# c-zhou/oatk

Measured on AMD Instinct MI355X. Metric: HiFi Gbases/s through syncasm (syncmer+syncerr) at k=1001 s=31, higher is better.
Workload: dtype u64

## Files before the change

oatk_amd/csrc/api_ec.inc:

```
#include "../../include/oatk_hip_ec.h"
#include "ec.hpp"
#include "ec_wave.hpp"
#include "ec_heavy.hpp"
#include "ec_fused.hpp"
#include "ecgraph.hpp"
#include "ec_seq.hpp"
#include <rocprim/device/device_run_length_encode.hpp>
#include <rocprim/device/device_select.hpp>

struct EcState {
    DevBuf idx_p, idx_n, arc_v, arc_w, arc_ls, arc_cov, arc_del, conv;
    DevBuf scm_del, err_del, vtx_hs_off, vtx_mpos;
    DevBuf copy_n, seg, keep_all, n_blocks, n_blocks64, blk_off, work, out, path_pool, cursor, todo, todo2, slabs, big_slabs, os_slabs;
    DevBuf hyb_slabs[16];
    hipStream_t aux[5] = {nullptr, nullptr, nullptr, nullptr, nullptr};
    hipEvent_t aux_ev[5] = {nullptr, nullptr, nullptr, nullptr, nullptr}, fork_ev = nullptr;
    DevBuf new_n, new_n64, new_off, new_k, new_m, new_s, stats;
    DevBuf live32, live64, live_off, larc, lidx_p, lidx_n;
    DevBuf cov, fwd, key_id, key_sorted, val_occ, occ, occ_off, cov64;
    uint64_t n_vtx = 0, new_tot = 0;
    uint64_t stats_h[12] = {0};
    uint64_t n_work = 0;
    bool done = false;
    DevBuf g_keys, g_keys2, g_ukeys, g_counts, g_nruns, g_nout, g_nout64, g_outoff, g_akey, g_aval, g_skey, g_sval, g_comp, g_flags, g_huge;
    DevBuf g_dist, g_dist2, g_cnt64, g_runoff, g_runls;
    DevBuf g_big, g_keep, g_other, g_lkeys, g_ldist, g_val2, g_wgt2, g_runcov, g_head, g_hpos, g_iota, g_segk, g_segv;
    uint32_t light_c = 0;
    uint64_t g_n_vtx = 0, g_n_arc = 0;
    bool graph_resident = false;
    bool global = false, marked = false;
    uint64_t n_global = 0, imp_used = 0;
    DevBuf g_l2g, g_kid, g_gcov, g_gs;
    bool keep_seq = false;
    bool seq_kept = false, cseq_done = false;
    bool seq_global = false;
    DevBuf slot_w, slot_w64, slot_off, slots, qend, sblk, clen, cbytes, cbytes64, coff, cseq;
    uint64_t cseq_bytes = 0;
};

static uint64_t ec_n_vtx(oatk_hip_ctx *ctx) { return ctx->ec && ctx->ec->global? ctx->ec->n_global : ctx->n_scm_total; }
static const uint64_t *ec_chains(oatk_hip_ctx *ctx) { return ctx->ec && ctx->ec->global? ctx->ec->g_kid.as<uint64_t>() : ctx->pos_kid.as<uint64_t>(); }

static void ec_state_free(oatk_hip_ctx *ctx)
{
    if (!ctx->ec) return;
    EcState *e = ctx->ec;
    for (int i = 0; i < 5; ++i) { if (e->aux[i]) (void) hipStreamDestroy(e->aux[i]); if (e->aux_ev[i]) (void) hipEventDestroy(e->aux_ev[i]); }
    if (e->fork_ev) (void) hipEventDestroy(e->fork_ev);
    delete e;
    ctx->ec = nullptr;
}

static int ec_buffer(oatk_hip_ctx *ctx, int which, const void **d_ptr, uint64_t *bytes)
{
    EcState *e = ctx->ec;
    if (e && which >= OATK_BUF_EG_IDX_P && which <= OATK_BUF_EG_ARC_COMP) {
        if (!e->graph_resident) { ctx->err = "EC graph requested before oatk_hip_ec_graph"; return OATK_E_STATE; }
        const uint64_t gv = e->g_n_vtx, ga = e->g_n_arc;
        switch (which) {
            case OATK_BUF_EG_IDX_P: *d_ptr = e->idx_p.p, *bytes = 2 * gv * 8; break;
            case OATK_BUF_EG_IDX_N: *d_ptr = e->idx_n.p, *bytes = 2 * gv * 4; break;
            case OATK_BUF_EG_ARC_V: *d_ptr = e->arc_v.p, *bytes = ga * 8; break;
            case OATK_BUF_EG_ARC_W: *d_ptr = e->arc_w.p, *bytes = ga * 8; break;
            case OATK_BUF_EG_ARC_LS: *d_ptr = e->arc_ls.p, *bytes = ga * 4; break;
            case OATK_BUF_EG_ARC_COV: *d_ptr = e->arc_cov.p, *bytes = ga * 4; break;
            default: *d_ptr = e->g_comp.p, *bytes = ga; break;
        }
        return OATK_OK;
    }
    if (e && (which == OATK_BUF_EC_VTX_SRC || (which == OATK_BUF_EC_ERR_DEL && !e->done))) {
        if (!e->marked) { ctx->err = "vertex sources / marks requested before oatk_hip_ec_mark"; return OATK_E_STATE; }
        if (which == OATK_BUF_EC_VTX_SRC) *d_ptr = e->vtx_hs_off.p, *bytes = e->n_vtx * 8;
        else *d_ptr = e->err_del.p, *bytes = e->n_vtx;
        return OATK_OK;
    }
// ... 576 lines not shown
{
    using namespace oatk;
    if (!ctx) return OATK_E_NODEV;
    if (!ctx->ec || !ctx->ec->marked) { ctx->err = "oatk_hip_ec_export_kmers needs oatk_hip_ec_mark"; return OATK_E_STATE; }
    if (stride % 16 || stride < (uint32_t) ((ctx->K + 3) / 4 + 8)) { ctx->err = "k-mer stride must be a multiple of 16 and hold the k-mer + 8 bytes"; return OATK_E_ARG; }
    CK(hipSetDevice(ctx->device));
    EcState *e = ctx->ec;
    if (n) hipLaunchKernelGGL(ecw_export_kmer_kernel, dim3((unsigned) n), dim3(64), 0, ctx->stream, n, d_ids, e->vtx_hs_off.as<uint64_t>(), e->vtx_mpos.as<uint32_t>(),
                              ctx->hoco_s.as<uint8_t>(), ctx->K, stride, d_out, d_rev);
    CK(hipStreamSynchronize(ctx->stream));
    CK(hipGetLastError());
    return OATK_OK;
}

extern "C" int oatk_hip_ec_import_kmers(oatk_hip_ctx *ctx, const uint32_t *d_ids, const uint8_t *d_rev, const uint8_t *d_kmers, uint64_t n, uint32_t stride)
{
    using namespace oatk;
    if (!ctx) return OATK_E_NODEV;
    if (!ctx->ec || !ctx->ec->marked) { ctx->err = "oatk_hip_ec_import_kmers needs oatk_hip_ec_mark"; return OATK_E_STATE; }
    if (stride % 16 || stride < (uint32_t) ((ctx->K + 3) / 4 + 8)) { ctx->err = "k-mer stride must be a multiple of 16 and hold the k-mer + 8 bytes"; return OATK_E_ARG; }
    CK(hipSetDevice(ctx->device));
    EcState *e = ctx->ec;
    if (n && !ctx->hoco_s.p) { ctx->err = "oatk_hip_ec_import_kmers: this batch has no hoco strings to put k-mers behind"; return OATK_E_STATE; }
    const uint64_t base = ((ctx->seq_bytes / 4 + 128) + 15) & ~15ULL;
    if (e->imp_used + n * stride > ctx->import_reserve) { ctx->err = "imported k-mers exceed the reserve behind the hoco strings (oatk_hip_ec_reserve_import before the scan)"; return OATK_E_NOMEM; }
    if (n) {
        CK(hipMemcpyAsync(ctx->hoco_s.as<uint8_t>() + base + e->imp_used, d_kmers, n * stride, hipMemcpyDeviceToDevice, ctx->stream));
        hipLaunchKernelGGL(ecw_import_kmer_kernel, dim3((unsigned) ((n + 255) / 256)), dim3(256), 0, ctx->stream, n, d_ids, d_rev, base + e->imp_used, stride,
                           e->vtx_hs_off.as<uint64_t>(), e->vtx_mpos.as<uint32_t>());
        e->imp_used += n * stride;
    }
    CK(hipStreamSynchronize(ctx->stream));
    CK(hipGetLastError());
    return OATK_OK;
}

extern "C" int oatk_hip_ec_reserve_import(oatk_hip_ctx *ctx, uint64_t bytes)
{
    if (!ctx) return OATK_E_NODEV;
    ctx->import_reserve = bytes < (1u << 20)? (1u << 20) : (bytes + 15) & ~15ULL;
    return OATK_OK;
}

struct EcKnobs {
    int heavy = -1;
    bool stages = false;
    bool serial_tiers = false;
    int32_t step_budget = 1000;
    int32_t min_nw = 0;
    int32_t heavy_cap2 = 0;
    int32_t heavy_fl = 0;
    int32_t waves = 32;
    bool assemble_walk = false;
};
static EcKnobs ec_knobs_read()
{
    EcKnobs k;
    auto num = [](const char *n, int32_t lo, int32_t dflt) { const char *e = getenv(n); return e && atoi(e) >= lo? (int32_t) atoi(e) : dflt; };
    { const char *e = getenv("OATK_DEBUG_EC_HEAVY"); k.heavy = e && (e[0] == '0' || e[0] == '1') && !e[1]? e[0] - '0' : -1; }
    k.stages = getenv("OATK_DEBUG_EC_STAGES") != nullptr;
    { const char *e = getenv("OATK_DEBUG_EC_SERIAL_TIERS"); k.serial_tiers = e && e[0] == '1'; }
    k.step_budget = num("OATK_DEBUG_EC_STEP_BUDGET", 1, 1000);
    k.min_nw = num("OATK_DEBUG_EC_FUSED_MIN_NW", 2, 0);
    k.heavy_cap2 = num("OATK_DEBUG_EC_HEAVY_CAP2", 1, 0), k.heavy_fl = num("OATK_DEBUG_EC_HEAVY_FL", 64, 0) & ~7;
    k.waves = num("OATK_DEBUG_EC_WAVES", 1, 32);
    { const char *e = getenv("OATK_DEBUG_EC_ASSEMBLE_WALK"); k.assemble_walk = e && e[0] == '1'; }
    return k;
}

namespace oatk {

static const int32_t EC_CAP_T0 = 3072;
static const int32_t EC_CAP_T1 = 16384;
static const int32_t EC_ARC_BUDGET = 512;

struct EcTier { int32_t cap_t, cap_c, cap_w, cap_path, cap_f; uint64_t bytes, slab; bool usable, hybrid; int wpb; };

static int32_t ec_cap_c(int32_t cap_t, int K) { return cap_t + cap_t / 8 + 2 * K + 64; }

static int32_t ec_band_cap(int32_t bwmax, double max_edist)
{
    int64_t ct = max_edist > 0? (int64_t) floor((double) bwmax / max_edist) : 0x3FFFFFFF;
    while (ct > 0 && (int32_t) ceil((double) ct * max_edist) > bwmax) --ct;
    return (int32_t) (ct > 60000? 60000 : ct);
}

static uint64_t ec_wg_per_cu(uint64_t bytes)
{
    const uint64_t n = 160 * 1024 / (bytes + 256);
    return n > 16? 16 : (n? n : 1);
}

static EcTier ec_lds_tier(int32_t cap_t, int32_t cap_path, int32_t cap_f, bool hybrid, double max_edist, int K)
{
    EcTier t;
    const int32_t bw = (int32_t) (cap_t * max_edist) + 1;
    t.cap_t = cap_t, t.cap_w = 2 * (bw > EC_MIN_ERR_BASE? bw : EC_MIN_ERR_BASE) + 12, t.cap_c = ec_cap_c(cap_t, K);
    t.hybrid = hybrid;
    if (hybrid) {
        t.cap_path = t.cap_c, t.cap_f = 1 << 20;
        t.bytes = (uint64_t) ecw_lds_words_hybrid(t.cap_t, t.cap_c, t.cap_w) * 4;
        t.slab = ecw_slab_bytes_hybrid(t.cap_path, t.cap_f);
    } else {
        t.cap_path = cap_path, t.cap_f = cap_f;
        t.bytes = (uint64_t) ecw_scratch_words(t.cap_t, t.cap_c, t.cap_w, t.cap_path, t.cap_f, false) * 4;
        t.slab = 0;
    }
    t.usable = t.bytes <= 64 * 1024;
    t.wpb = ECW_WPB * t.bytes <= 64 * 1024? ECW_WPB : 1;
    return t;
}

static uint64_t ec_tier_waves(const EcTier &t, int32_t per_cu_max, int n_cu)
{
    uint64_t per_cu = ec_wg_per_cu((uint64_t) t.wpb * t.bytes) * (uint64_t) t.wpb;
    if (per_cu > (uint64_t) per_cu_max) per_cu = (uint64_t) per_cu_max / (uint64_t) t.wpb * (uint64_t) t.wpb;
    return (uint64_t) n_cu * (per_cu? per_cu : (uint64_t) t.wpb);
}

// ... 345 lines not shown
    int used_aux = 0;
    if (side_by_side) {
        { int rc = ec_route(ctx, e, n_work, rt, routed, sizeof(routed)); if (rc) return rc; }
        { int rc = ec_fork_side_streams(ctx, e); if (rc) return rc; }
        for (int tier = LAST - 1; tier >= 1; --tier) {
            if (!T[tier].usable || !routed[tier]) continue;
            hipStream_t st = e->aux[used_aux];
            CK(hipStreamWaitEvent(st, e->fork_ev, 0));
            { int rc = launch(tier, list[tier], routed[tier], st, true, tier == 1? 2 * (uint64_t) ctx->n_cu : 0); if (rc) return rc; }
            CK(hipEventRecord(e->aux_ev[used_aux], st));
            ++used_aux;
            done[tier] = routed[tier];
        }
    }
    const int first_tier = side_by_side || T[0].usable? 0 : next_usable(0);
    { int rc = launch(first_tier, nullptr, 0, ctx->stream, side_by_side); if (rc) return rc; }
    bool waited_aux = used_aux == 0;
    for (int round = 0; ; ++round) {
        CK(hipMemcpyAsync(cnts, cur, sizeof(cnts), hipMemcpyDeviceToHost, ctx->stream));
        CK(hipStreamSynchronize(ctx->stream));
        if (round == 0) n_big = cnts[1] + cnts[2] + routed[3];
        bool any = false;
        for (int tier = first_tier + 1; tier <= LAST; ++tier) {
            if (!T[tier].usable || cnts[tier] <= done[tier]) continue;
            { int rc = launch(tier, list[tier] + done[tier], cnts[tier] - done[tier], ctx->stream, false); if (rc) return rc; }
            done[tier] = cnts[tier];
            any = true;
        }
        if (!any && waited_aux) break;
        if (!waited_aux) { for (int i = 0; i < used_aux; ++i) CK(hipStreamWaitEvent(ctx->stream, e->aux_ev[i], 0)); waited_aux = true; }
    }
    return OATK_OK;
}

}

extern "C" int oatk_hip_ec_correct(oatk_hip_ctx *ctx, double max_edist)
{
    using namespace oatk;
    if (!ctx) return OATK_E_NODEV;
    if (!ctx->ec || !ctx->ec->marked) { ctx->err = "oatk_hip_ec_correct needs oatk_hip_ec_mark"; return OATK_E_STATE; }
    CK(hipSetDevice(ctx->device));
    EcState *e = ctx->ec;
    e->done = false, e->cseq_done = false;
    const bool keep_seq = e->keep_seq;
    e->seq_kept = false;
    const EcKnobs kn = ec_knobs_read();
    EC_VIEWS();
    EcLive lv;
    bool graph_branches = true;
    {
        uint64_t n_live = 0;
        EENSURE(g_flags, 64);
        CK(hipMemsetAsync(e->g_flags.as<uint32_t>() + 8, 0, 8, ctx->stream));
        EENSURE(live32, (na + 1) * 4); EENSURE(lidx_p, (2 * nv + 1) * 4); EENSURE(lidx_n, (2 * nv + 1) * 4);
        if (na) hipLaunchKernelGGL(ec_live_flag_kernel, blocks(na), dim3(256), 0, ctx->stream, na, (const uint8_t *) e->arc_del.p, e->live32.as<uint32_t>());
        { int rc = ec_exclusive_scan_u32(ctx, e, e->live32, e->live64, e->live_off, na, &n_live); if (rc) return rc; }
        if (n_live >= 0xFFFFFFFFULL) { ctx->err = "error correction: more than 2^32 live arcs"; return OATK_E_ARG; }
        EENSURE(larc, (n_live + 1) * sizeof(EcLiveArc));
        hipLaunchKernelGGL(ec_live_idx_kernel, blocks(2 * nv), dim3(256), 0, ctx->stream, 2 * nv, e->idx_p.as<uint64_t>(), e->idx_n.as<uint32_t>(),
                           e->live_off.as<uint64_t>(), e->lidx_p.as<uint32_t>(), e->lidx_n.as<uint32_t>(), e->g_flags.as<uint32_t>() + 9);
        if (na) hipLaunchKernelGGL(ec_live_arc_kernel, blocks(na), dim3(256), 0, ctx->stream, na, (const uint8_t *) e->arc_del.p, e->live_off.as<uint64_t>(),
                                   e->arc_w.as<uint64_t>(), e->arc_ls.as<uint32_t>(), e->vtx_hs_off.as<uint64_t>(), e->vtx_mpos.as<uint32_t>(),
                                   e->lidx_p.as<uint32_t>(), e->lidx_n.as<uint32_t>(), e->larc.as<EcLiveArc>(), e->g_flags.as<uint32_t>() + 8);
        uint32_t fl[2] = {0, 0};
        CK(hipMemcpyAsync(fl, e->g_flags.as<uint32_t>() + 8, 8, hipMemcpyDeviceToHost, ctx->stream));
        CK(hipStreamSynchronize(ctx->stream));
        const uint32_t no_src = fl[0];
        graph_branches = fl[1] != 0;
        if (no_src && ctx->n_occ) { ctx->err = "error correction: a live vertex has no k-mer on this shard (import it: oatk_hip_ec_import_kmers)"; return OATK_E_STATE; }
        lv.idx_p = e->lidx_p.as<uint32_t>(), lv.idx_n = e->lidx_n.as<uint32_t>(), lv.arc = e->larc.as<EcLiveArc>();
    }

    EENSURE(n_blocks, (nr + 1) * 4);
    const dim3 rblocks((unsigned) ((nr + ECR_READS_PER_BLOCK - 1) / ECR_READS_PER_BLOCK > 0? (nr + ECR_READS_PER_BLOCK - 1) / ECR_READS_PER_BLOCK : 1));
    hipLaunchKernelGGL(ec_count_blocks_wave_kernel, rblocks, dim3(256), 0, ctx->stream, rd, (const uint8_t *) e->scm_del.p, e->n_blocks.as<uint32_t>());
    uint64_t n_work = 0;
    { int rc = ec_exclusive_scan_u32(ctx, e, e->n_blocks, e->n_blocks64, e->blk_off, nr, &n_work); if (rc) return rc; }
    EENSURE(work, (n_work + 1) * sizeof(EcWork)); EENSURE(out, (n_work + 1) * sizeof(EcBlockOut));
    e->n_work = n_work;
    EENSURE(new_n, (nr + 1) * 4); EENSURE(copy_n, (nr + 1) * 4); EENSURE(seg, (n_work + 1) * sizeof(EcSeg)); EENSURE(keep_all, nr + 1);
    hipLaunchKernelGGL(ec_list_blocks_wave_kernel, rblocks, dim3(256), 0, ctx->stream, rd, lv, (const uint8_t *) e->scm_del.p, e->blk_off.as<uint64_t>(), e->work.as<EcWork>(), e->copy_n.as<uint32_t>(),
                       e->seg.as<EcSeg>(), e->keep_all.as<uint8_t>());
    if (keep_seq) {
        uint64_t slot_words = 0;
        EENSURE(slot_w, (n_work + 1) * 4); EENSURE(qend, (n_work + 1) * 4);
        if (n_work) hipLaunchKernelGGL(ec_slot_words_kernel, blocks(n_work), dim3(256), 0, ctx->stream, e->work.as<EcWork>(), n_work, max_edist, e->slot_w.as<uint32_t>());
        { int rc = ec_exclusive_scan_u32(ctx, e, e->slot_w, e->slot_w64, e->slot_off, n_work, &slot_words); if (rc) return rc; }
        EENSURE(slots, (slot_words + 4) * 4);
    }
    t_end(ctx, OATK_T_EC_MARK);
    t_begin(ctx, OATK_T_EC_SOLVE);

    const bool heavy = kn.heavy < 0? graph_branches : kn.heavy != 0;
    uint64_t pool_cap = 2 * nocc + (uint64_t) 16384 * ECW_POOL_CHUNK + 4096;
    EENSURE(cursor, 512); EENSURE(stats, 16 * 8);
    uint64_t n_big = 0;
    uint32_t max_hl = 0;
    for (;;) {
        EENSURE(path_pool, pool_cap * 8);
        CK(hipMemsetAsync(e->cursor.p, 0, 512, ctx->stream));
        EcwArgs base = {};
        base.lv = lv, base.rd = rd, base.work = e->work.as<EcWork>(), base.n_work = n_work, base.max_edist = max_edist;
        base.out = e->out.as<EcBlockOut>(), base.path_pool = e->path_pool.as<uint64_t>(), base.pool_cap = pool_cap;
        base.pool_cursor = (unsigned long long *) e->cursor.p;
        if (keep_seq) {
            CK(hipMemsetAsync(e->qend.p, 0, (n_work + 1) * 4, ctx->stream));
            base.seq_qend = e->qend.as<uint32_t>(), base.seq_slots = e->slots.as<uint32_t>(), base.seq_slot_off = e->slot_off.as<uint64_t>();
        }
        if (kn.stages) fprintf(stderr, "[ec stages] the live graph %s: %s\n", graph_branches? "branches" : "does not branch", heavy? "classes with budgets, second stage" : "round 4's tiers");
        { int rc = heavy? ec_solve_classes(ctx, e, kn, base, max_hl, n_big) : ec_solve_tiers(ctx, e, kn, base, max_hl, n_big); if (rc) return rc; }
        unsigned long long fin = 0, used = 0;
        CK(hipMemcpyAsync(&fin, base.pool_cursor + 63, 8, hipMemcpyDeviceToHost, ctx->stream));
        CK(hipStreamSynchronize(ctx->stream));
        if (fin) { ctx->err = "error correction: a block outgrew the large scratch slab (DFS deeper than 4 MiB of frames)"; return OATK_E_NOMEM; }
        CK(hipMemcpyAsync(&used, e->cursor.p, 8, hipMemcpyDeviceToHost, ctx->stream));
        CK(hipStreamSynchronize(ctx->stream));
        if (used <= pool_cap) break;
        pool_cap = used + used / 4 + 4096;
    }

    t_end(ctx, OATK_T_EC_SOLVE);
    t_begin(ctx, OATK_T_EC_REFRESH);
    EENSURE(new_n, (nr + 1) * 4);
    CK(hipMemsetAsync(e->stats.p, 0, 16 * 8, ctx->stream));
    EcAssembleArgs aa;
    aa.rd = rd, aa.scm_del = (const uint8_t *) e->scm_del.p, aa.scm_s = g.scm_s, aa.blk_off = e->blk_off.as<uint64_t>();
    aa.out = e->out.as<EcBlockOut>(), aa.path_pool = e->path_pool.as<uint64_t>(), aa.new_n = e->new_n.as<uint32_t>(), aa.new_off = nullptr;
    aa.new_k_mer = nullptr, aa.new_s_mer = nullptr, aa.new_m_pos = nullptr, aa.old_s_mer = ctx->pos_smer.as<uint64_t>();
    aa.stats = (unsigned long long *) e->stats.p, aa.pass = 1, aa.seg = e->seg.as<EcSeg>(), aa.keep_all = e->keep_all.as<uint8_t>();
    if (n_work) hipLaunchKernelGGL(ec_block_stats_kernel, dim3((unsigned) (n_work / 256 + 1 < 512? n_work / 256 + 1 : 512)), dim3(256), 0, ctx->stream, e->work.as<EcWork>(),
                                   e->out.as<EcBlockOut>(), n_work, (unsigned long long *) e->stats.p);
    if (kn.assemble_walk) hipLaunchKernelGGL(ec_new_n_kernel, blocks(nr), dim3(256), 0, ctx->stream, nr, e->copy_n.as<uint32_t>(), e->blk_off.as<uint64_t>(), e->work.as<EcWork>(), e->out.as<EcBlockOut>(), e->new_n.as<uint32_t>());
    else hipLaunchKernelGGL(ec_new_n_seg_kernel, blocks(nr), dim3(256), 0, ctx->stream, nr, e->copy_n.as<uint32_t>(), e->blk_off.as<uint64_t>(), e->seg.as<EcSeg>(), e->out.as<EcBlockOut>(), e->new_n.as<uint32_t>());
    uint64_t tot = 0;
    { int rc = ec_exclusive_scan_u32(ctx, e, e->new_n, e->new_n64, e->new_off, nr, &tot); if (rc) return rc; }
// ... 136 lines not shown
```

oatk_amd/csrc/ec.hpp:

```cpp
#pragma once
#include "common.hpp"

namespace oatk {

#define EC_FAILURE 0
#define EC_SUCCESS 1
#define EC_AMBISNQ 2
#define EC_AMBISEQ 3
#define EC_MAX_DFS_PATH 10000
#define EC_MIN_ERR_SEQ_LEN 10
#define EC_MIN_ERR_BASE 6
#define EC_NONE 0xFFFFFFFFFFFFFFFFULL

struct EcGraph {
    uint64_t n_vtx, n_arc;
    const uint64_t *idx_p;
    const uint32_t *idx_n;
    const uint64_t *arc_v, *arc_w;
    const uint32_t *arc_ls, *arc_cov;
    uint8_t *arc_del;
    uint8_t *scm_del;
    const uint32_t *scm_cov;
    const uint64_t *scm_s;
    const uint64_t *vtx_hs_off;
// ... 330 lines not shown
        if (lane == 0) n_blocks[x.r] = (uint32_t) nb;
    }
}

__global__ __launch_bounds__(256) void ec_list_blocks_wave_kernel(EcReads rd, EcLive lv, const uint8_t *scm_del, const uint64_t *blk_off, EcWork *work, uint32_t *copy_n, EcSeg *seg,
                                                                  uint8_t *keep_all)
{
    const uint64_t r0 = ((uint64_t) blockIdx.x * 4 + (threadIdx.x >> 6)) * ECR_RPW;
    const int lane = threadIdx.x & 63;
    if (r0 >= rd.n_reads) return;
    EcrRead q[ECR_RPW];
    ecr_load(rd, scm_del, r0, lane, q);
    EcWork *wq[ECR_RPW];
    EcSeg *sq[ECR_RPW];
    uint32_t hq[ECR_RPW];
#pragma unroll
    for (int k = 0; k < ECR_RPW; ++k) {
        const uint64_t b0 = q[k].n >= 0? blk_off[q[k].r] : 0;
        wq[k] = q[k].n >= 0? work + b0 : nullptr, sq[k] = q[k].n >= 0? seg + b0 : nullptr, hq[k] = q[k].n >= 0? (uint32_t) (rd.off[q[k].r] >> 6) : 0u;
    }
#pragma unroll
    for (int k = 0; k < ECR_RPW; ++k) {
        const EcrRead &x = q[k];
        if (x.n < 0) continue;
        EcWork *w = wq[k];
        EcSeg *sg = sq[k];
        const uint32_t hs16 = hq[k];
        const int32_t n = x.n;
        auto put = [&](int i, const EcBlock &b) {
            EcWork y;
            y.beg_utg = b.beg_utg, y.end_utg = b.end_utg, y.read = (uint32_t) x.r, y.beg_pos = b.beg_pos, y.l = b.l, y.r = b.r;
            y.hs16 = hs16, y.lp = lv.idx_p[b.beg_utg], y.ln = lv.idx_n[b.beg_utg];
            const int32_t last = b.end < n? b.end : n;
            y.pad = b.r? (uint32_t) b.beg : (b.beg + 1 < n && last > b.beg + 1? (uint32_t) (last - b.beg - 1) : 0u);
            w[i] = y;
            sg[i] = ec_seg_of(b, n);
        };
        uint32_t cp = 0;
        auto on_copy = [&](int32_t first, int32_t last) { if (last > first) cp += (uint32_t) (last - first); };
        if (x.n > 64) {
            if (lane == 0) {
                const int nbs = ec_blocks(scm_del, rd.k_mer + x.o, rd.m_pos + x.o, x.n, x.hoco_l, rd.K, put, on_copy);
                copy_n[x.r] = nbs < 0? (uint32_t) n : cp;
                keep_all[x.r] = nbs < 0;
            }
            continue;
        }
        EcBlock mine;
        mine.beg_utg = 0, mine.end_utg = 0, mine.beg_pos = 0, mine.l = 0, mine.beg = 0, mine.end = 0, mine.r = 0;
        const int nb = ec_blocks_wave(lane, x.n, x.km, x.mp, x.del, x.hoco_l, rd.K,
                                      [&](int i, const EcBlock &b) { if (i < 64) { if (lane == i) mine = b; } else if (lane == 0) put(i, b); }, on_copy);
        if (lane < nb) put(lane, mine);
        if (lane == 0) copy_n[x.r] = nb < 0? (uint32_t) n : cp, keep_all[x.r] = nb < 0;
    }
}

__global__ __launch_bounds__(256) void ec_new_n_kernel(uint64_t n_reads, const uint32_t *copy_n, const uint64_t *blk_off, const EcWork *work, const EcBlockOut *out, uint32_t *new_n)
{
    const uint64_t r = (uint64_t) blockIdx.x * blockDim.x + threadIdx.x;
    if (r >= n_reads) return;
    uint32_t s = copy_n[r];
    for (uint64_t i = blk_off[r]; i < blk_off[r + 1]; ++i) {
        if (out[i].status == EC_SUCCESS) {
            const int32_t np = (int32_t) out[i].np;
            s += work[i].r? (uint32_t) (np >= 1? np - 1 : 0) : (uint32_t) ((np >= 2? np - 2 : 0) + (work[i].end_utg == EC_NONE && np > 1? 1 : 0));
        } else s += work[i].pad;
    }
    new_n[r] = s;
}

__global__ __launch_bounds__(256) void ec_block_stats_kernel(const EcWork *work, const EcBlockOut *out, uint64_t n_work, unsigned long long *stats)
{
    __shared__ uint32_t part[4][11];
    uint32_t loc[11] = {0, 0, 0, 0, 0, 0, 0, 0, 0, 0, 0};
    for (uint64_t i = (uint64_t) blockIdx.x * blockDim.x + threadIdx.x; i < n_work; i += (uint64_t) gridDim.x * blockDim.x) {
        const EcBlockOut x = out[i];
        if (x.short_block) ++loc[10];
        else if (work[i].end_utg == EC_NONE) ++loc[0], ++loc[1 + x.status];
        else ++loc[5], ++loc[6 + x.status];
    }
    for (int i = 0; i < 11; ++i) {
        uint32_t v = loc[i];
        for (int d = 32; d; d >>= 1) v += __shfl_xor(v, d);
        if ((threadIdx.x & 63) == 0) part[threadIdx.x >> 6][i] = v;
    }
    __syncthreads();
    if (threadIdx.x < 11) {
        const uint32_t v = part[0][threadIdx.x] + part[1][threadIdx.x] + part[2][threadIdx.x] + part[3][threadIdx.x];
        if (v) atomicAdd(&stats[threadIdx.x], (unsigned long long) v);
    }
}

__device__ inline void ec_assemble_read_serial(const EcAssembleArgs &a, uint64_t r)
{
    const uint64_t o = a.rd.scm_off[r];
    const int32_t n = (int32_t) (a.rd.scm_off[r + 1] - o);
    const uint64_t *km = a.rd.k_mer + o;
    const uint32_t *mp = a.rd.m_pos + o;
    const EcBlockOut *bo = a.out + a.blk_off[r];
    uint64_t wpos = a.pass? a.new_off[r] : 0;
    const uint64_t w0 = wpos;
    uint32_t cnt = 0;
    auto put = [&](uint64_t k, uint32_t m) {
        if (a.pass) {
            a.new_k_mer[wpos] = k, a.new_m_pos[wpos] = m, a.new_s_mer[wpos] = a.scm_s[k >> 1];
            a.key_id[wpos] = (uint32_t) (k >> 1), a.val_occ[wpos] = (a.sid0 + r) << 32 | (wpos - w0) << 1 | (m & 1u);
// ... 243 lines not shown
```

oatk_amd/csrc/scan_syncmer_fast.hpp:

```cpp
#pragma once
#include <type_traits>
#include "common.hpp"
#include "scan_syncmer.hpp"
#include "scan_hpc.hpp"

namespace oatk {

constexpr int SYF_C = 8;
constexpr int SYF_T = SYN_NT * SYF_C;
constexpr int SYF_BLK = 64;
constexpr int SYF_LIST = 128;

static inline int syncmer_fast_ring(int K, int S)
{
    const int w = K - S;
    if (w / SYF_C - 1 < SYF_BLK || w / SYF_C - 1 >= 2 * SYF_BLK) return 0;
    if (K + SYF_T + SYF_C + 64 <= 4096) return 4096;
    return 0;
}

#define OATK_DPP_ROW_SHL(n) (0x100 + (n))
#define OATK_DPP_ROW_SHR(n) (0x110 + (n))
#define OATK_DPP_ROW_BCAST15 0x142
#define OATK_DPP_ROW_BCAST31 0x143
// ... 120 lines not shown
#pragma unroll
        for (int ww = 0; ww < NWAVE; ++ww) { const uint32_t c = w_cnt[pend_par][ww]; tot += c; before += ww < (int) wid? c : 0u; }
        pend_any = 0;
        if (tot == 0) return;
        if (sl_n + tot > lcap) emit_list();
        const bool direct = tot > lcap;
        if (direct) {
            if (tid == 0) s_gb = atomicAdd(&a.shard_cnt[blockIdx.x & (OATK_REC_SHARDS - 1)], tot);
            __syncthreads();
            uint32_t rank = before + pend_rank, kk = pend_kinds;
            while (kk) {
                const int o = __builtin_ctz(kk) >> 1;
                const uint32_t kind = (pend_kinds >> (2 * o)) & 3u;
                kk &= ~(3u << (2 * o));
                write_record(pend_i0 + o, kind, s_gb + rank, ord0 + rank);
                ++rank;
            }
            __syncthreads();
        } else if (pend_wtot) {
            uint32_t idx = sl_n + before + pend_rank, kk = pend_kinds;
            while (kk) {
                const int o = __builtin_ctz(kk) >> 1;
                sl_e[idx] = (uint32_t) (pend_i0 + o) | ((pend_kinds >> (2 * o)) & 3u) << 30;
                kk &= ~(3u << (2 * o));
                ++idx;
            }
        }
        ord0 += direct? tot : 0u;
        sl_n += direct? 0u : tot;
    };

    static_assert(2 * T == R, "the address toggling below needs tile = half the ring");
    struct RangeAddr { uint32_t lo, hi, mid; bool whole; };
    auto range_addr = [&](int32_t lo, int32_t hi) -> RangeAddr {
        return RangeAddr{rch(lo) * 4u, rch(hi) * 4u, rch(((lo >> 6) + 1) * 64 + 63) * 4u, (hi >> 6) - (lo >> 6) == 2};
    };
    const int32_t ch_0 = (int32_t) tid, ca0_0 = ((int32_t) (tid * C) - w) >> 3;
    RangeAddr rB = range_addr(ch_0 - D, ch_0 - 1), rF0 = range_addr(ca0_0 + 1, ca0_0 + D), rF1 = range_addr(ca0_0 + 2, ca0_0 + 1 + D);
    uint32_t o_cs = rch(ch_0) * 4u;
    uint32_t m_own = mi((int32_t) (tid * C)), m_fa = mi(ca0_0 * C), m_fb = mi((ca0_0 + 1) * C);
    const uint32_t m_own_sum = m_own + mi((int32_t) (tid * C) + T), m_fa_sum = m_fa + mi(ca0_0 * C + T), m_fb_sum = m_fb + mi((ca0_0 + 1) * C + T);
    auto next_tile_addr = [&]() __attribute__((always_inline)) {
        constexpr uint32_t FLIP = (uint32_t) (NCH / 2) * 4u;
        o_cs ^= FLIP;
        rB.lo ^= FLIP, rB.hi ^= FLIP, rB.mid ^= FLIP, rF0.lo ^= FLIP, rF0.hi ^= FLIP, rF0.mid ^= FLIP, rF1.lo ^= FLIP, rF1.hi ^= FLIP, rF1.mid ^= FLIP;
        m_own = m_own_sum - m_own, m_fa = m_fa_sum - m_fa, m_fb = m_fb_sum - m_fb;
    };
    auto ld32 = [](const uint32_t *base, uint32_t byte_off) -> uint32_t { return *(const uint32_t *) ((const char *) base + byte_off); };

    bool rep_mode = false, rep_next = false;
    int32_t rep_start = 0x7FFFFFFF;
    uint32_t quiet = 0, tpar = 0;
    const int32_t wave_first = __builtin_amdgcn_readfirstlane((int) (wid * OATK_WAVE * C));
    for (uint32_t I0 = 0; I0 < hl; I0 += T, next_tile_addr(), tpar ^= 1u) {
        if (rep_next != rep_mode) { rep_mode = rep_next; rep_start = rep_mode? (int32_t) (I0 / C) : 0x7FFFFFFF; }
        const int32_t i0 = (int32_t) (I0 + tid * C);
        const int32_t wb = (int32_t) I0 + wave_first;
        const int32_t ch = i0 / C;
        uint32_t y[C];
        uint32_t cmin_keep;
        {
            const uint32_t a_hi = __builtin_amdgcn_perm(rw0, rw1, bsel), a_lo = __builtin_amdgcn_perm(rw1, rw2, bsel);
            const uint32_t vbh = __builtin_amdgcn_perm(rw2, 0u, bsel);
            const uint64_t vb = (uint64_t) vbh << 32;
            {
                const uint32_t wn = ((I0 + T + tid * C) - 32u) >> 4;
                const Words3 nx = *(const Words3 *) (ghs + (wn < last_w? wn : last_w));
                rw0 = nx.a, rw1 = nx.b, rw2 = nx.c;
            }
            uint64_t cm = UINT64_MAX;
            uint32_t cmin = 0xFFFFFFFFu;
            if (wb + 1 >= S && (uint32_t) (wb + OATK_WAVE * C) <= hl) {
                if (S31) {
                    auto rc16 = [](uint32_t x) -> uint32_t {
                        const uint32_t r = __builtin_bitreverse32(x);
                        return ~(((r >> 1) & 0x55555555u) | ((r & 0x55555555u) << 1));
                    };
                    const uint32_t r0 = rc16(a_hi), r1 = rc16(a_lo), r2 = rc16(vbh);
                    auto hash_chunk = [&](auto keep) __attribute__((always_inline)) {
#pragma unroll
                        for (int b = 0; b < C; ++b) {
                            uint64_t fw = (uint64_t) __builtin_amdgcn_alignbit(a_hi, a_lo, 28 - 2 * b) << 32 | __builtin_amdgcn_alignbit(a_lo, vbh, 28 - 2 * b);
                            uint64_t rv = (uint64_t) __builtin_amdgcn_alignbit(r2, r1, 2 + 2 * b) << 32 | __builtin_amdgcn_alignbit(r1, r0, 2 + 2 * b);
                            asm("" : "+v"(fw), "+v"(rv));
                            const uint64_t cn = fw < rv? fw : rv;
                            const uint64_t mv4 = hash64_s31_left(cn);
                            y[b] = (uint32_t) (mv4 >> 34);
                            cmin = y[b] < cmin? y[b] : cmin;
                            if (decltype(keep)::value) cm = mv4 < cm? mv4 : cm;
                        }
                        if (decltype(keep)::value) cm >>= 2;
                    };
                    if (__builtin_amdgcn_readfirstlane((int) rep_mode)) hash_chunk(std::true_type()); else hash_chunk(std::false_type());
                } else {
                    const uint64_t X = ((uint64_t) a_hi << 32 | a_lo) << (2 * (32 - S));
                    uint64_t fw = X >> (64 - 2 * S), rv = revcomp32(X) & mask;
#pragma unroll
                    for (int b = 0; b < C; ++b) {
                        const uint64_t c = (vbh >> (30 - 2 * b)) & 3u;
                        fw = (fw << 2 | c) & mask;
                        rv = rv >> 2 | (3ULL ^ c) << (2 * S - 2);
                        const uint64_t mv = fw != rv? hash64(fw < rv? fw : rv, mask) : UINT64_MAX;
                        y[b] = (uint32_t) (mv >> 32);
                        cmin = y[b] < cmin? y[b] : cmin;
                        cm = mv < cm? mv : cm;
                    }
                }
            } else {
                const uint64_t X = ((uint64_t) a_hi << 32 | a_lo) << (2 * (32 - S));
                uint64_t fw = X >> (64 - 2 * S), rv = revcomp32(X) & mask;
#pragma unroll
                for (int b = 0; b < C; ++b) {
                    const int32_t i = i0 + b;
                    const uint64_t c = (vb >> (62 - 2 * b)) & 3ULL;
                    fw = (fw << 2 | c) & mask;
                    rv = rv >> 2 | (3ULL ^ c) << (2 * S - 2);
                    uint64_t mv = UINT64_MAX;
                    if (i + 1 >= S && (uint32_t) i < hl && fw != rv) mv = S31? hash64_s31(fw < rv? fw : rv) : hash64(fw < rv? fw : rv, mask);
                    y[b] = (uint32_t) (mv >> 32);
                    cmin = y[b] < cmin? y[b] : cmin;
                    if (rep_mode) cm = mv < cm? mv : cm;
                }
            }
            cmin_keep = cmin;
            uint32_t pre, suf;
#ifdef OATK_SCAN_SHFL
            pre = suf = cmin;
            for (int d = 1; d < OATK_WAVE; d <<= 1) {
                uint32_t up = __shfl_up(pre, d), dn = __shfl_down(suf, d);
                if ((int) lane >= d) pre = up < pre? up : pre;
                if ((int) lane + d < OATK_WAVE) suf = dn < suf? dn : suf;
            }
#else
            pre = wave_prefix_min_u32(cmin);
            suf = wave_suffix_min_mirrored_u32(cmin, lane);
#endif
            __syncthreads();
            static_assert(C == 8, "two 16-byte stores per lane");
            *(uint4 *) (m_top + m_own) = make_uint4(y[0], y[1], y[2], y[3]);
            *(uint4 *) (m_top + m_own + 4) = make_uint4(y[4], y[5], y[6], y[7]);
            if (rep_mode) *(uint64_t *) ((char *) c_min + 2u * o_cs) = cm;
            {
                const uint32_t seen = s_tie[tpar ^ 1u];
                quiet = seen? 0u : quiet + 1u;
                rep_next = seen != 0u || (rep_mode && quiet < 2u);
            }
            *(uint32_t *) ((char *) pre32 + o_cs) = pre;
#ifdef OATK_SCAN_SHFL
            *(uint32_t *) ((char *) suf32 + o_cs) = suf;
#else
            *(uint32_t *) ((char *) suf32 + (o_cs ^ 252u)) = suf;
#endif
        }
        __syncthreads();
        if (tid == 0) s_tie[tpar ^ 1u] = 0;
        flush();

        static_assert(SH >= 0 && SH < C, "the window's alignment against the chunks is a template argument");
        constexpr int RR = (C - SH) & (C - 1);
        uint32_t backF_keep = 0, fwd0_keep = 0, fwd1_keep = 0;
        uint32_t kinds = 0;
        uint32_t tiemask = 0;
        {
            auto range_min = [&](const RangeAddr &ra) -> uint32_t {
                const uint32_t a0 = ld32(suf32, ra.lo), a1 = ld32(pre32, ra.hi);
                const uint32_t mid = ld32(pre32, ra.mid);
                const uint32_t a2 = ra.whole? mid : 0xFFFFFFFFu;
                const uint32_t v = a0 < a1? a0 : a1;
                return a2 < v? a2 : v;
            };
            const uint32_t backF = range_min(rB);
            const uint32_t fwd0 = range_min(rF0);
            const uint32_t fwd1 = range_min(rF1);
            backF_keep = backF, fwd0_keep = fwd0, fwd1_keep = fwd1;
            constexpr int BD = RR? RR : C;
            uint32_t W[2 * C];
            {
                const uint4 a0 = *(const uint4 *) (m_top + m_fa), a1 = *(const uint4 *) (m_top + m_fa + 4);
                const uint4 b0 = *(const uint4 *) (m_top + m_fb), b1 = *(const uint4 *) (m_top + m_fb + 4);
                const uint32_t all[2 * C] = {a0.x, a0.y, a0.z, a0.w, a1.x, a1.y, a1.z, a1.w, b0.x, b0.y, b0.z, b0.w, b1.x, b1.y, b1.z, b1.w};
#pragma unroll
                for (int j = 0; j < 2 * C - SH; ++j) W[j] = all[SH + j];
            }
            uint32_t cprev = 0xFFFFFFFFu;
            if (RR > 0) {
                const uint32_t nb = dpp_u32<0x138>(0xFFFFFFFFu, cmin_keep);
                const uint32_t lb = ld32(suf32, (o_cs - 4u) & (uint32_t) (NCH * 4 - 1));
                cprev = lane == 0? lb : nb;
            }
            const bool edge = !(wb + 1 >= K && (uint32_t) (wb + OATK_WAVE * C) <= hl);
            auto decide = [&](auto at_edge) __attribute__((always_inline)) {
#pragma unroll
                for (int o = 0; o < C; ++o) {
                    const uint32_t yhi = y[o], fhi = W[o];
                    const uint32_t fb = o + SH < C? fwd0 : fwd1;
                    const uint32_t fy = fb < yhi? fb : yhi;
                    const bool c1 = yhi <= backF, c2 = fhi <= fy;
                    uint64_t cand = __ballot(c1) | __ballot(c2);
                    bool fits = true;
                    if (decltype(at_edge)::value) {
                        fits = (uint32_t) (i0 + o) < hl && i0 + o + 1 >= K;
                        cand &= __ballot(fits);
                    }
#if OATK_SYF_EXP == 1
                    if (!a.want_n) cand = 0;
#endif
                    if (cand) {
                        const bool c = (c1 | c2) && fits;
                        uint32_t pmin = 0xFFFFFFFFu;
#pragma unroll
                        for (int j = 0; j < o; ++j) pmin = y[j] < pmin? y[j] : pmin;
                        const int cend = o < BD? BD - 1 : BD + C - 1;
                        uint32_t rest = 0xFFFFFFFFu;
#pragma unroll
                        for (int j = o + 1; j <= cend; ++j) rest = W[j] < rest? W[j] : rest;
                        uint32_t head = fhi < rest? fhi : rest;
// ... 33 lines not shown
            auto full = [&](int32_t q, uint32_t ref) -> uint64_t {
                const uint32_t t = m_top[mi(q)];
                return t == ref? hash_at(q) : (uint64_t) t << 32;
            };
            uint64_t r0 = UINT64_MAX, r1 = UINT64_MAX;
            if (tiemask) {
                const int32_t ca0 = (i0 - w) >> 3;
                uint64_t mid = UINT64_MAX;
                for (int32_t cc = ca0 + 2; cc <= ca0 + D; ++cc) { const uint64_t u = c_min[rch(cc)]; mid = u < mid? u : mid; }
                const uint64_t e0 = c_min[rch(ca0 + 1)], e1 = c_min[rch(ca0 + 1 + D)];
                r0 = e0 < mid? e0 : mid, r1 = e1 < mid? e1 : mid;
            }
            const uint64_t r_close = (w & (C - 1))? r1 : r0;
            uint32_t tm = tiemask;
            while (tm) {
                const int o = __builtin_ctz(tm);
                tm &= tm - 1;
                const int32_t E = i0 + o, lo = E - w;
                const uint32_t yhi = m_top[mi(E)], fhi = m_top[mi(lo)];
                const uint64_t yy = hash_at(E), f = hash_at(lo);
                const uint32_t fb = o + sh < C? fwd0_keep : fwd1_keep;
                bool cl = false, op = false;
                if (yhi <= backF_keep) {
                    uint64_t b = UINT64_MAX;
                    for (int t = 0; t < HW - o; ++t) { const uint64_t u = t? full(lo + t, yhi) : f; b = u < b? u : b; }
                    for (int t = 0; t < o; ++t) { const uint64_t u = full(i0 + t, yhi); b = u < b? u : b; }
                    if (yhi == backF_keep) b = r_close < b? r_close : b;
                    if (yy != UINT64_MAX && yy <= b) {
                        const uint64_t x = full(lo - 1, yhi);
                        cl = yy < b || x >= b || f == b;
                    }
                }
                if (fhi <= fb && fhi <= yhi) {
                    const int32_t ca = lo >> 3, tail0 = (ca + 1 + D) * C;
                    uint64_t b = UINT64_MAX;
                    for (int32_t q = lo + 1; q < (ca + 1) * C; ++q) { const uint64_t u = full(q, fhi); b = u < b? u : b; }
                    for (int32_t q = tail0; q < E; ++q) { const uint64_t u = full(q, fhi); b = u < b? u : b; }
                    if (fhi == fb) { const uint64_t u = ca == ((i0 - w) >> 3)? r0 : r1; b = u < b? u : b; }
                    op = f != UINT64_MAX && f <= b && f <= yy;
                }
                kinds |= (cl && op? 0u : (cl? 1u : (op? 2u : 0u))) << (2 * o);
            }
        }
#if OATK_SYF_EXP == 5
        kinds &= (uint32_t) -a.want_n;
#endif
        const uint32_t ns = (uint32_t) __builtin_popcount((kinds | kinds >> 1) & 0x5555u);
        const uint32_t incl = wave_incl_sum_dpp(ns, lane);
        const uint32_t wtot = (uint32_t) __builtin_amdgcn_readlane((int) incl, 63);
        if (lane == 0) w_cnt[par][wid] = wtot;
        pend_kinds = kinds, pend_rank = incl - ns, pend_i0 = i0, pend_wtot = wtot, pend_par = par, pend_any = 1u;
        par ^= 1u;
    }
    __syncthreads();
    flush();
    __syncthreads();
    emit_list();
    if (tid == 0) a.n_scm[r] = ord0;
}

}
```

Measured before the change: 375.6.

## Stage error blocks in one walk and trim syncmer scan edge work

Error-block enumeration used to walk each read twice, once to count blocks and once to list them. It now walks once, writes each block into a per-read staging array sized syncmers+1, and a separate fill kernel builds the work entries from it after the scan, with an overflow flag checked on the host. The syncmer scan also stops early for waves past the read end, handles edge chunks on the fast S=31 path with per-base masking instead of the slow path, and skips range-min work for tiles entirely before K. The cost is extra staging memory, an extra device-to-host copy, and added barrier bookkeeping for waves that exit early.

Result: faster. 382.9, median of 6 (+1.9%).

```diff
diff --git a/oatk_amd/csrc/api_ec.inc b/oatk_amd/csrc/api_ec.inc
--- a/oatk_amd/csrc/api_ec.inc
+++ b/oatk_amd/csrc/api_ec.inc
@@ -21,6 +21,7 @@
     uint64_t n_vtx = 0, new_tot = 0;
     uint64_t stats_h[12] = {0};
     uint64_t n_work = 0;
+    uint32_t staged_over = 0;
     bool done = false;
     DevBuf g_keys, g_keys2, g_ukeys, g_counts, g_nruns, g_nout, g_nout64, g_outoff, g_akey, g_aval, g_skey, g_sval, g_comp, g_flags, g_huge;
     DevBuf g_dist, g_dist2, g_cnt64, g_runoff, g_runls;
@@ -703,6 +704,7 @@
     int32_t heavy_fl = 0;
     int32_t waves = 32;
     bool assemble_walk = false;
+    bool list_walk = false;
 };
 static EcKnobs ec_knobs_read()
 {
@@ -716,6 +718,7 @@
     k.heavy_cap2 = num("OATK_DEBUG_EC_HEAVY_CAP2", 1, 0), k.heavy_fl = num("OATK_DEBUG_EC_HEAVY_FL", 64, 0) & ~7;
     k.waves = num("OATK_DEBUG_EC_WAVES", 1, 32);
     { const char *e = getenv("OATK_DEBUG_EC_ASSEMBLE_WALK"); k.assemble_walk = e && e[0] == '1'; }
+    { const char *e = getenv("OATK_DEBUG_EC_LIST_WALK"); k.list_walk = e && e[0] == '1'; }
     return k;
 }
 
@@ -1167,7 +1170,7 @@
     {
         uint64_t n_live = 0;
         EENSURE(g_flags, 64);
-        CK(hipMemsetAsync(e->g_flags.as<uint32_t>() + 8, 0, 8, ctx->stream));
+        CK(hipMemsetAsync(e->g_flags.as<uint32_t>() + 8, 0, 12, ctx->stream));
         EENSURE(live32, (na + 1) * 4); EENSURE(lidx_p, (2 * nv + 1) * 4); EENSURE(lidx_n, (2 * nv + 1) * 4);
         if (na) hipLaunchKernelGGL(ec_live_flag_kernel, blocks(na), dim3(256), 0, ctx->stream, na, (const uint8_t *) e->arc_del.p, e->live32.as<uint32_t>());
         { int rc = ec_exclusive_scan_u32(ctx, e, e->live32, e->live64, e->live_off, na, &n_live); if (rc) return rc; }
@@ -1189,14 +1192,26 @@
 
     EENSURE(n_blocks, (nr + 1) * 4);
     const dim3 rblocks((unsigned) ((nr + ECR_READS_PER_BLOCK - 1) / ECR_READS_PER_BLOCK > 0? (nr + ECR_READS_PER_BLOCK - 1) / ECR_READS_PER_BLOCK : 1));
-    hipLaunchKernelGGL(ec_count_blocks_wave_kernel, rblocks, dim3(256), 0, ctx->stream, rd, (const uint8_t *) e->scm_del.p, e->n_blocks.as<uint32_t>());
+    EENSURE(new_n, (nr + 1) * 4); EENSURE(copy_n, (nr + 1) * 4); EENSURE(keep_all, nr + 1);
+    const uint64_t stage_cap = nocc + nr + 1;
+    e->staged_over = 0;
+    if (kn.list_walk) hipLaunchKernelGGL(ec_count_blocks_wave_kernel, rblocks, dim3(256), 0, ctx->stream, rd, (const uint8_t *) e->scm_del.p, e->n_blocks.as<uint32_t>());
+    else {
+        static_assert(sizeof(EcSeg) == 8, "a staging entry is one val_occ entry");
+        EENSURE(val_occ, stage_cap * sizeof(EcSeg));
+        hipLaunchKernelGGL(ec_stage_blocks_wave_kernel, rblocks, dim3(256), 0, ctx->stream, rd, (const uint8_t *) e->scm_del.p, e->n_blocks.as<uint32_t>(), e->copy_n.as<uint32_t>(),
+                           e->keep_all.as<uint8_t>(), e->val_occ.as<EcSeg>(), stage_cap, e->g_flags.as<uint32_t>() + 10);
+        CK(hipMemcpyAsync(&e->staged_over, e->g_flags.as<uint32_t>() + 10, 4, hipMemcpyDeviceToHost, ctx->stream));
+    }
     uint64_t n_work = 0;
     { int rc = ec_exclusive_scan_u32(ctx, e, e->n_blocks, e->n_blocks64, e->blk_off, nr, &n_work); if (rc) return rc; }
+    if (e->staged_over) { ctx->err = "error correction: a read has more error blocks than syncmers + 1 (the block walk's staging array)"; return OATK_E_STATE; }
     EENSURE(work, (n_work + 1) * sizeof(EcWork)); EENSURE(out, (n_work + 1) * sizeof(EcBlockOut));
     e->n_work = n_work;
-    EENSURE(new_n, (nr + 1) * 4); EENSURE(copy_n, (nr + 1) * 4); EENSURE(seg, (n_work + 1) * sizeof(EcSeg)); EENSURE(keep_all, nr + 1);
-    hipLaunchKernelGGL(ec_list_blocks_wave_kernel, rblocks, dim3(256), 0, ctx->stream, rd, lv, (const uint8_t *) e->scm_del.p, e->blk_off.as<uint64_t>(), e->work.as<EcWork>(), e->copy_n.as<uint32_t>(),
-                       e->seg.as<EcSeg>(), e->keep_all.as<uint8_t>());
+    EENSURE(seg, (n_work + 1) * sizeof(EcSeg));
+    if (kn.list_walk) hipLaunchKernelGGL(ec_list_blocks_wave_kernel, rblocks, dim3(256), 0, ctx->stream, rd, lv, (const uint8_t *) e->scm_del.p, e->blk_off.as<uint64_t>(), e->work.as<EcWork>(),
+                                         e->copy_n.as<uint32_t>(), e->seg.as<EcSeg>(), e->keep_all.as<uint8_t>());
+    else hipLaunchKernelGGL(ec_fill_work_kernel, blocks(nr), dim3(256), 0, ctx->stream, rd, lv, e->blk_off.as<uint64_t>(), (const EcSeg *) e->val_occ.as<EcSeg>(), e->work.as<EcWork>(), e->seg.as<EcSeg>());
     if (keep_seq) {
         uint64_t slot_words = 0;
         EENSURE(slot_w, (n_work + 1) * 4); EENSURE(qend, (n_work + 1) * 4);
diff --git a/oatk_amd/csrc/ec.hpp b/oatk_amd/csrc/ec.hpp
--- a/oatk_amd/csrc/ec.hpp
+++ b/oatk_amd/csrc/ec.hpp
@@ -406,6 +406,87 @@
                                       [&](int i, const EcBlock &b) { if (i < 64) { if (lane == i) mine = b; } else if (lane == 0) put(i, b); }, on_copy);
         if (lane < nb) put(lane, mine);
         if (lane == 0) copy_n[x.r] = nb < 0? (uint32_t) n : cp, keep_all[x.r] = nb < 0;
+    }
+}
+
+__global__ __launch_bounds__(256) void ec_stage_blocks_wave_kernel(EcReads rd, const uint8_t *scm_del, uint32_t *n_blocks, uint32_t *copy_n, uint8_t *keep_all, EcSeg *stage,
+                                                                   uint64_t stage_cap, uint32_t *overflow)
+{
+    const uint64_t r0 = ((uint64_t) blockIdx.x * 4 + (threadIdx.x >> 6)) * ECR_RPW;
+    const int lane = threadIdx.x & 63;
+    if (r0 >= rd.n_reads) return;
+    EcrRead q[ECR_RPW];
+    ecr_load(rd, scm_del, r0, lane, q);
+#pragma unroll
+    for (int k = 0; k < ECR_RPW; ++k) {
+        const EcrRead &x = q[k];
+        if (x.n < 0) continue;
+        const int32_t n = x.n;
+        const uint64_t s0 = x.o + x.r;
+        auto put = [&](int i, const EcBlock &b) {
+            if (i <= n && s0 + (uint64_t) i < stage_cap) stage[s0 + (uint64_t) i] = ec_seg_of(b, n); else *overflow = 1u;
+        };
+        uint32_t cp = 0;
+        auto on_copy = [&](int32_t first, int32_t last) { if (last > first) cp += (uint32_t) (last - first); };
+        if (n > 64) {
+            if (lane == 0) {
+                const int nbs = ec_blocks(scm_del, rd.k_mer + x.o, rd.m_pos + x.o, n, x.hoco_l, rd.K, put, on_copy);
+                n_blocks[x.r] = nbs < 0? 0u : (uint32_t) nbs;
+                copy_n[x.r] = nbs < 0? (uint32_t) n : cp;
+                keep_all[x.r] = nbs < 0;
+            }
+            continue;
+        }
+        EcBlock mine;
+        mine.beg_utg = 0, mine.end_utg = 0, mine.beg_pos = 0, mine.l = 0, mine.beg = 0, mine.end = 0, mine.r = 0;
+        int nb = 0;
+        const int res = ec_blocks_wave(lane, n, x.km, x.mp, x.del, x.hoco_l, rd.K,
+                                       [&](int i, const EcBlock &b) { ++nb; if (i < 64) { if (lane == i) mine = b; } else if (lane == 0) put(i, b); }, on_copy);
+        if (lane < nb) put(lane, mine);
+        if (lane == 0) n_blocks[x.r] = (uint32_t) nb, copy_n[x.r] = res < 0? (uint32_t) n : cp, keep_all[x.r] = res < 0;
+    }
+}
+
+__device__ __forceinline__ EcWork ec_work_of(const EcReads &rd, const EcLive &lv, uint64_t r, uint64_t o, int32_t n, const EcSeg &d)
+{
+    const int32_t beg = (int32_t) d.beg, end = (int32_t) (d.end_fl >> 2);
+    const uint64_t kb = rd.k_mer[o + d.beg];
+    const uint32_t mb = rd.m_pos[o + d.beg];
+    EcWork y;
+    y.read = (uint32_t) r, y.hs16 = (uint32_t) (rd.off[r] >> 6);
+    if (d.end_fl & EC_SEG_R) {
+        y.beg_utg = (kb & ~1ULL) | (uint64_t) !(mb & 1u);
+        y.beg_pos = 0, y.end_utg = EC_NONE, y.l = (int32_t) (mb >> 1), y.r = 1;
+        y.pad = d.beg;
+    } else {
+        y.beg_utg = (kb & ~1ULL) | (mb & 1u);
+        y.beg_pos = (mb >> 1) + (uint32_t) rd.K;
+        if (d.end_fl & EC_SEG_OPEN) y.end_utg = EC_NONE, y.l = (int32_t) rd.hoco_l[r] - (int32_t) y.beg_pos;
+        else {
+            const uint64_t ke = rd.k_mer[o + (uint32_t) end];
+            const uint32_t me = rd.m_pos[o + (uint32_t) end];
+            y.end_utg = (ke & ~1ULL) | (me & 1u), y.l = (int32_t) (me >> 1) - (int32_t) y.beg_pos;
+        }
+        y.r = 0;
+        y.pad = beg + 1 < n && end > beg + 1? (uint32_t) (end - beg - 1) : 0u;
+    }
+    y.lp = lv.idx_p[y.beg_utg], y.ln = lv.idx_n[y.beg_utg];
+    return y;
+}
+
+__global__ __launch_bounds__(256) void ec_fill_work_kernel(EcReads rd, EcLive lv, const uint64_t *blk_off, const EcSeg *stage, EcWork *work, EcSeg *seg)
+{
+    __shared__ uint64_t offs[257];
+    const uint64_t r0 = (uint64_t) blockIdx.x * 256;
+    for (uint32_t t = threadIdx.x; t < 257; t += 256) offs[t] = blk_off[r0 + t < rd.n_reads? r0 + t : rd.n_reads];
+    __syncthreads();
+    for (uint64_t j = offs[0] + threadIdx.x; j < offs[256]; j += 256) {
+        uint32_t lo = 0, hi = 256;
+        while (hi - lo > 1) { const uint32_t mid = (lo + hi) >> 1; if (offs[mid] <= j) lo = mid; else hi = mid; }
+        const uint64_t r = r0 + lo, o = rd.scm_off[r];
+        const EcSeg d = stage[o + r + (j - offs[lo])];
+        work[j] = ec_work_of(rd, lv, r, o, (int32_t) (rd.scm_off[r + 1] - o), d);
+        seg[j] = d;
     }
 }
 
diff --git a/oatk_amd/csrc/scan_syncmer_fast.hpp b/oatk_amd/csrc/scan_syncmer_fast.hpp
--- a/oatk_amd/csrc/scan_syncmer_fast.hpp
+++ b/oatk_amd/csrc/scan_syncmer_fast.hpp
@@ -196,7 +196,8 @@
     int32_t rep_start = 0x7FFFFFFF;
     uint32_t quiet = 0, tpar = 0;
     const int32_t wave_first = __builtin_amdgcn_readfirstlane((int) (wid * OATK_WAVE * C));
-    for (uint32_t I0 = 0; I0 < hl; I0 += T, next_tile_addr(), tpar ^= 1u) {
+    uint32_t I0 = 0;
+    for (; I0 + (uint32_t) wave_first < hl; I0 += T, next_tile_addr(), tpar ^= 1u) {
         if (rep_next != rep_mode) { rep_mode = rep_next; rep_start = rep_mode? (int32_t) (I0 / C) : 0x7FFFFFFF; }
         const int32_t i0 = (int32_t) (I0 + tid * C);
         const int32_t wb = (int32_t) I0 + wave_first;
@@ -214,28 +215,38 @@
             }
             uint64_t cm = UINT64_MAX;
             uint32_t cmin = 0xFFFFFFFFu;
-            if (wb + 1 >= S && (uint32_t) (wb + OATK_WAVE * C) <= hl) {
+            const bool inside = wb + 1 >= S && (uint32_t) (wb + OATK_WAVE * C) <= hl;
+            if (S31 || inside) {
                 if (S31) {
                     auto rc16 = [](uint32_t x) -> uint32_t {
                         const uint32_t r = __builtin_bitreverse32(x);
                         return ~(((r >> 1) & 0x55555555u) | ((r & 0x55555555u) << 1));
                     };
                     const uint32_t r0 = rc16(a_hi), r1 = rc16(a_lo), r2 = rc16(vbh);
-                    auto hash_chunk = [&](auto keep) __attribute__((always_inline)) {
+                    auto hash_chunk = [&](auto keep, auto ends) __attribute__((always_inline)) {
 #pragma unroll
                         for (int b = 0; b < C; ++b) {
                             uint64_t fw = (uint64_t) __builtin_amdgcn_alignbit(a_hi, a_lo, 28 - 2 * b) << 32 | __builtin_amdgcn_alignbit(a_lo, vbh, 28 - 2 * b);
                             uint64_t rv = (uint64_t) __builtin_amdgcn_alignbit(r2, r1, 2 + 2 * b) << 32 | __builtin_amdgcn_alignbit(r1, r0, 2 + 2 * b);
                             asm("" : "+v"(fw), "+v"(rv));
                             const uint64_t cn = fw < rv? fw : rv;
-                            const uint64_t mv4 = hash64_s31_left(cn);
+                            uint64_t mv4 = hash64_s31_left(cn);
                             y[b] = (uint32_t) (mv4 >> 34);
+                            if (decltype(ends)::value) {
+                                const bool ok = i0 + b + 1 >= S && (uint32_t) (i0 + b) < hl;
+                                y[b] = ok? y[b] : 0xFFFFFFFFu;
+                                if (decltype(keep)::value) mv4 = ok? mv4 : UINT64_MAX;
+                            }
                             cmin = y[b] < cmin? y[b] : cmin;
                             if (decltype(keep)::value) cm = mv4 < cm? mv4 : cm;
                         }
-                        if (decltype(keep)::value) cm >>= 2;
+                        if (decltype(keep)::value) cm = decltype(ends)::value && cm == UINT64_MAX? cm : cm >> 2;
                     };
-                    if (__builtin_amdgcn_readfirstlane((int) rep_mode)) hash_chunk(std::true_type()); else hash_chunk(std::false_type());
+                    if (inside) {
+                        if (__builtin_amdgcn_readfirstlane((int) rep_mode)) hash_chunk(std::true_type(), std::false_type()); else hash_chunk(std::false_type(), std::false_type());
+                    } else {
+                        if (__builtin_amdgcn_readfirstlane((int) rep_mode)) hash_chunk(std::true_type(), std::true_type()); else hash_chunk(std::false_type(), std::true_type());
+                    }
                 } else {
                     const uint64_t X = ((uint64_t) a_hi << 32 | a_lo) << (2 * (32 - S));
                     uint64_t fw = X >> (64 - 2 * S), rv = revcomp32(X) & mask;
@@ -305,7 +316,7 @@
         uint32_t backF_keep = 0, fwd0_keep = 0, fwd1_keep = 0;
         uint32_t kinds = 0;
         uint32_t tiemask = 0;
-        {
+        if (!(wb + OATK_WAVE * C < K)) {
             auto range_min = [&](const RangeAddr &ra) -> uint32_t {
                 const uint32_t a0 = ld32(suf32, ra.lo), a1 = ld32(pre32, ra.hi);
                 const uint32_t mid = ld32(pre32, ra.mid);
@@ -445,6 +456,13 @@
         pend_kinds = kinds, pend_rank = incl - ns, pend_i0 = i0, pend_wtot = wtot, pend_par = par, pend_any = 1u;
         par ^= 1u;
     }
+    if (I0 < hl) {
+        __syncthreads();
+        __syncthreads();
+        flush();
+        if (lane == 0) w_cnt[par][wid] = 0;
+        pend_kinds = 0, pend_rank = 0, pend_wtot = 0, pend_par = par, pend_any = 1u;
+    }
     __syncthreads();
     flush();
     __syncthreads();
```
